# yukiteruono/pbsim3

Measured on AMD Instinct MI355X. Metric: simulated bases/sec, higher is better.
Workload: dtype u8

## Files before the change

pbsim3_amd/csrc/job.cpp:

```cpp
#include <math.h>
#include <stdio.h>
#include <stdlib.h>
#include <string.h>

#include <algorithm>
#include <atomic>
#include <chrono>
#include <condition_variable>
#include <deque>
#include <future>
#include <mutex>
#include <thread>

#include "ctx.h"
#include "handoff.h"

using namespace pbsim;

namespace {

double now_us() {
  return std::chrono::duration<double, std::micro>(std::chrono::steady_clock::now().time_since_epoch()).count();
}

constexpr double kMinBatchBases = 2.0e9;
constexpr int kRoundsPerRecord = 4;

struct Rec {
  RefDesc ref;
  int64_t quota = 0, len_total = 0, next_read = 1, spec_read = 1;
  double spec_total = 0;
  int64_t cap = 0;
  bool bulk_done = false;
  bool done = false;
  int owner = -1;
  int tail_slot = -1;
  bool tail_waiting = false;
  int64_t read_off = 0, maf_off = 0;
  int64_t tail_read = 0, tail_maf = 0;
  StatsAcc st;
  bool merged = false;
};

struct Round {
  int rec, slot;
  int64_t first, n_per;
  double mean;
  bool clear;
};

struct Worker {
  std::thread th;
  std::mutex mu;
  std::condition_variable cv, cv_idle;
  std::deque<std::function<void()>> q;
  bool stop = false, running = false;
  int active = 0;
  struct Deferred {
    int key;
    std::function<bool()> ready;
    std::function<void()> run;
  };
  std::deque<Deferred> parked;
  int n_parked = 0;
  void defer(int key, std::function<bool()> ready, std::function<void()> run) {
    parked.push_back(Deferred{key, std::move(ready), std::move(run)});
    std::lock_guard<std::mutex> lk(mu);
    n_parked++;
  }
  bool run_parked() {
    bool any = false;
    for (size_t i = 0; i < parked.size();) {
      bool first_of_key = true;
      for (size_t j = 0; j < i; j++) first_of_key &= parked[j].key != parked[i].key;
      if (first_of_key && parked[i].ready()) {
        Deferred d = std::move(parked[i]);
        parked.erase(parked.begin() + (long)i);
        d.run();
        {
          std::lock_guard<std::mutex> lk(mu);
          n_parked--;
        }
        any = true;
        i = 0;
      } else {
        i++;
      }
    }
    return any;
  }
  void start(int device) {
    running = true;
    th = std::thread([this, device]() {
      (void)hipSetDevice(device);
      for (;;) {
        std::function<void()> f;
        {
          std::unique_lock<std::mutex> lk(mu);
          if (parked.empty()) cv.wait(lk, [&] { return stop || !q.empty(); });
          else cv.wait_for(lk, std::chrono::milliseconds(1), [&] { return stop || !q.empty(); });
          if (q.empty() && parked.empty()) return;
          if (!q.empty()) {
            f = std::move(q.front());
            q.pop_front();
            active++;
          }
        }
        if (f) {
          f();
          std::lock_guard<std::mutex> lk(mu);
          active--;
        }
        if (run_parked() || f) cv_idle.notify_all();
      }
    });
  }
  void post(std::function<void()> f) {
    {
      std::lock_guard<std::mutex> lk(mu);
      q.push_back(std::move(f));
    }
    cv.notify_one();
  }
  void drain() {
    if (!running) return;
    std::unique_lock<std::mutex> lk(mu);
    cv_idle.wait(lk, [&] { return q.empty() && active == 0 && n_parked == 0; });
  }
  void finish() {
    if (!running) return;
    drain();
    {
      std::lock_guard<std::mutex> lk(mu);
      stop = true;
    }
    cv.notify_all();
    th.join();
    running = false;
  }
  ~Worker() { finish(); }
};

struct Delivery {
  int slot = -1, rec = -1;
  bool mine = false;
  int64_t n_per = 0;
  std::shared_ptr<std::promise<int>> stage1;
  std::future<int> stage1_done;
  int64_t sizes[2] = {0, 0};
  int ok1 = PBSIM_SUCCEEDED;
  double t_wait0 = 0, t_wait1 = 0;
};

struct Job {
  pbsim_ctx *c;
  const pbsim_comm *comm;
  const pbsim_record_sink *sink;
  int rank = 0, W = 1;
  bool multi = false;
  std::vector<Rec> recs;
  std::deque<Round> fifo;
  double mean = 0;
  int depth = 3;
  int interleave = 1;
  int64_t reads_walked = 0, reads_delivered = 0, rounds = 0, bases = 0, ref_bases = 0, maf_columns = 0;
  double comm_us = 0;
  double bd_wait_walk = 0, bd_finalize = 0, bd_wait_bytes = 0, bd_account = 0, bd_tail_block = 0, bd_drain = 0, bd_slot_wait = 0,
         bd_merge = 0, bd_begin = 0, bd_tail_steps = 0;
  double bd_worker_busy = 0;
  int64_t n_topup = 0, n_tail_reads = 0, n_clear_missed = 0, n_exchanges = 0;
  bool trace = false;
  double t_start = 0;
  bool peer_failed = false;
  Worker worker;
  Worker tail_worker;
  std::mutex sink_mu[2];
  std::mutex out_mu;
  std::condition_variable out_cv;
  std::atomic<bool> delivering[kMaxSlots];
  std::atomic<bool> wfailed{false};
  std::mutex werr_mu;
  std::string werr;
  std::unique_ptr<Delivery> pending;
  std::unique_ptr<std::atomic<int>[]> rec_out;
  std::unique_ptr<std::atomic<int>[]> rec_bulk;
  std::unique_ptr<std::atomic<int>[]> rec_rounds_open;
  void round_closed(int rec) {
    --rec_rounds_open[(size_t)rec];
    { std::lock_guard<std::mutex> lk(out_mu); }
    out_cv.notify_all();
  }
  std::atomic<bool> giving_up{false};
  void wait_record(int rec) {
    std::unique_lock<std::mutex> lk(out_mu);
    out_cv.wait(lk, [&] { return rec_out[(size_t)rec].load() == 0; });
  }
  void delivered_one(std::atomic<int> *out, std::atomic<int> *bulk = nullptr) {
    --*out;
    if (bulk) --*bulk;
    { std::lock_guard<std::mutex> lk(out_mu); }
    out_cv.notify_all();
  }

  Job() {
    for (auto &d : delivering) d = false;
  }

  size_t n_collected = 0;
  bool seen11 = false;
  double bd_record_wait = 0;
  const DeviceFlags *record_arrived(int i) {
    JobRecord *jr = nullptr;
    {
      std::unique_lock<std::mutex> lk(c->job_mu);
      const double t0 = now_us();
      const bool came = c->job_cv.wait_for(lk, std::chrono::seconds(600),
                                           [&] { return c->job_records.size() > (size_t)i || c->job_feed_failed; });
      bd_record_wait += now_us() - t0;
      if (c->job_records.size() <= (size_t)i) {
        fail(!came ? "pbsim_job_run: a record announced by pbsim_job_expect did not arrive within 600 s" : c->job_feed_err);
        return nullptr;
      }
      jr = c->job_records[(size_t)i].get();
    }
    const double t1 = now_us();
    if (hipEventSynchronize(jr->ready) != hipSuccess) {
      fail("hipEventSynchronize failed (a record's preparation)");
      return nullptr;
// ... 5 lines not shown
    while ((int)n_collected <= upto) {
      const size_t i = n_collected;
      const DeviceFlags *f = record_arrived((int)i);
      if (!f) return PBSIM_FAILED;
      JobRecord *jr;
      {
        std::lock_guard<std::mutex> lk(c->job_mu);
        jr = c->job_records[i].get();
      }
      if (trace) fprintf(stderr, "[pbsim job r%d] t=%.1f ms record %zu collected (waited %.1f ms for records so far)\n", rank, (now_us() - t_start) / 1e3, i + 1, bd_record_wait / 1e3);
      seen11 |= f->hpfreq[11] > 0;
      jr->ref.seq = jr->seq.as<uint8_t>();
      jr->ref.hp = jr->hp.as<uint8_t>();
      jr->ref.len = jr->len;
      jr->ref.unit = c->job_first_unit + (int64_t)i;
      jr->ref.hp_flag = c->p.hp_del_bias == 1 && !f->high_bytes;
      jr->ref.hp11 = seen11;
      recs[i].ref = jr->ref;
      c->bias.hp11_seen = seen11;
      if (!ensure_tables(c, jr->ref.hp11)) return PBSIM_FAILED;
      n_collected++;
    }
    return PBSIM_SUCCEEDED;
  }

  void worker_fail() {
    std::lock_guard<std::mutex> lk(werr_mu);
    if (!wfailed) werr = g_err;
    wfailed = true;
  }
  int check_worker() {
    if (!wfailed) return PBSIM_SUCCEEDED;
    std::lock_guard<std::mutex> lk(werr_mu);
    return fail(werr);
  }

  void progress(int phase, int rec, int64_t first = 0, int64_t n_per = 0) {
    int64_t *g = c->job_progress;
    g[0] = phase;
    g[1] = rec;
    g[2] = first;
    g[3] = n_per;
    g[4] = W;
    g[5] = rec >= 0 ? recs[(size_t)rec].len_total : 0;
    g[6] = rec >= 0 ? recs[(size_t)rec].quota : 0;
    g[7] = rec >= 0 ? recs[(size_t)rec].next_read : 0;
  }
  int gather(const int64_t *send, int64_t n, std::vector<int64_t> *recv) {
    recv->assign((size_t)W * n, 0);
    if (!multi) {
      memcpy(recv->data(), send, (size_t)n * 8);
      return PBSIM_SUCCEEDED;
    }
    const double t0 = now_us();
    const int ok = comm->all_gather_i64(comm->user, send, n, recv->data());
    comm_us += now_us() - t0;
    n_exchanges++;
    return ok ? PBSIM_SUCCEEDED : fail("pbsim_comm.all_gather_i64 failed");
  }

  bool slot_busy(int s) const {
    if (delivering[s]) return true;
    for (const Round &r : fifo)
      if (r.slot == s) return true;
    for (const Rec &r : recs)
      if (r.tail_slot == s) return true;
    return false;
  }
  static constexpr int kTailSlot = kMaxSlots - 2;
  int free_slot() const {
    for (int s = 0; s < kTailSlot; s++)
      if (!slot_busy(s)) return s;
    return -1;
  }
  int free_tail_slot() const {
    for (int s = kTailSlot; s < kMaxSlots; s++)
      if (!slot_busy(s)) return s;
    return -1;
  }
  int bulk_in_flight() const { return (int)fifo.size(); }
  int acquire_slot() {
    const double t0 = now_us();
    for (;;) {
      const int s = free_slot();
      if (s >= 0) {
        bd_slot_wait += now_us() - t0;
        return s;
      }
      std::unique_lock<std::mutex> lk(worker.mu);
      worker.cv_idle.wait_for(lk, std::chrono::milliseconds(2));
    }
  }

  void drop_round(const Round &r) {
    c->cur = r.slot;
    (void)hipStreamSynchronize(c->s().stream);
    (void)settle_slot(r.slot);
    c->s().b_enqueued = false;
  }
  void drop_rounds_of(int rec) {
    for (auto it = fifo.begin(); it != fifo.end();) {
      if (it->rec == rec) {
        drop_round(*it);
        it = fifo.erase(it);
      } else {
        ++it;
      }
    }
  }
  void drop_everything(bool failing = true) {
    if (failing) {
      giving_up = true;
      { std::lock_guard<std::mutex> lk(out_mu); }
      out_cv.notify_all();
    }
    worker.drain();
    tail_worker.drain();
    for (const Round &r : fifo) drop_round(r);
    fifo.clear();
    for (Rec &r : recs)
      if (r.tail_slot >= 0) {
        c->cur = r.tail_slot;
        (void)hipStreamSynchronize(c->s().stream);
        c->s().b_enqueued = false;
        r.tail_slot = -1;
      }
  }

  Handoff handoff;
  bool handoff_on = false;
  bool lookahead = false;
  int64_t n_handed = 0, n_handed_void = 0;
  void publish_next(int slot) {
    const Slot &sl = c->slots[slot];
    if (!handoff_on || sl.b_info.n_final <= 0) return;
    HandoffNext d;
    d.slot = slot;
    d.text[0] = sink->on_read_text ? sl.d_read_text.p : nullptr;
    d.text[1] = sink->on_maf_text ? sl.d_maf_text.p : nullptr;
    d.bytes[0] = sl.b_info.read_text_bytes;
    d.bytes[1] = sl.b_info.maf_text_bytes;
    d.ev_text = sl.ev_text;
    handoff.publish(d);
  }
  unsigned withdraw_next() {
    if (!handoff_on) return 0;
    const unsigned took = handoff.withdraw();
    n_handed += (took & 1) + (took >> 1);
    return took;
  }
  int settle_slot(int slot) {
    for (DfLane &L : c->slots[slot].df) {
      if (L.hand_open) n_handed_void++;
      if (!deflate_settle(L)) return PBSIM_FAILED;
    }
    return PBSIM_SUCCEEDED;
  }
  std::function<bool()> tail_hook(int which) {
    return [this, which]() -> bool {
      return handoff.take(which, [&](const HandoffNext &d) {
        if (!d.text[which] || d.bytes[which] <= 0) return;
        (void)deflate_handoff(c, c->slots[d.slot].df[which], which, (const uint8_t *)d.text[which], d.bytes[which], !multi,
                              (hipEvent_t)d.ev_text);
      });
    };
  }

// ... 64 lines not shown
      }, nullptr, handoff_on ? &hook : nullptr);
    });
  }
  int arena_fill(Slot &sl, int64_t *read_gz, int64_t *maf_gz) {
    const pbsim_batch_info &bi = sl.b_info;
    *read_gz = *maf_gz = 0;
    return both_lanes(sl, [&](int which) -> int {
      DfLane &L = sl.df[which];
      L.arena_reset();
      const int64_t n = which == 0 ? bi.read_text_bytes : bi.maf_text_bytes;
      auto cb = which == 0 ? sink->on_read_text : sink->on_maf_text;
      if (!cb || n == 0) return PBSIM_SUCCEEDED;
      const uint8_t *d = which == 0 ? sl.d_read_text.as<uint8_t>() : sl.d_maf_text.as<uint8_t>();
      bool oom = false;
      const std::function<char *(int64_t)> place = [&](int64_t k) -> char * {
        char *p = L.arena_reserve(k, arena_max);
        if (!p) oom = true;
        return p;
      };
      const std::function<bool()> hook = tail_hook(which);
      if (!deflate_pieces(c, L, d, n, [](const char *, int64_t) { return PBSIM_SUCCEEDED; }, &place, handoff_on ? &hook : nullptr))
        return oom ? fail("out of pinned host memory for a compressed batch (PBSIM_PINNED_ARENA_MB bounds a lane's arena)") : PBSIM_FAILED;
      int64_t tot = 0;
      for (const auto &sg : L.arena_segs) tot += sg.second;
      (which == 0 ? *read_gz : *maf_gz) = tot;
      return PBSIM_SUCCEEDED;
    });
  }
  int arena_flush(Slot &sl, int64_t unit, int64_t read_at, int64_t maf_at) {
    return both_lanes(sl, [&](int which) -> int {
      int64_t at = which == 0 ? read_at : maf_at;
      for (const auto &sg : sl.df[which].arena_segs) {
        if (!call_sink(which, unit, sg.first, sg.second, at)) return fail(which == 0 ? "sink aborted (read text)" : "sink aborted (MAF text)");
        at += sg.second;
      }
      sl.df[which].arena_segs.clear();
      return PBSIM_SUCCEEDED;
    });
  }

  void submit_stage1(Delivery *d) {
    d->stage1 = std::make_shared<std::promise<int>>();
    d->stage1_done = d->stage1->get_future();
    if (!d->mine) {
      d->stage1->set_value(PBSIM_SUCCEEDED);
      return;
    }
    delivering[d->slot] = true;
    Slot *sl = &c->slots[d->slot];
    Rec *R = &recs[(size_t)d->rec];
    auto prom = d->stage1;
    int64_t *sizes = d->sizes;
    const int64_t read_at = R->read_off, maf_at = R->maf_off;
    std::atomic<int> *out = &rec_out[(size_t)d->rec], *bulk = &rec_bulk[(size_t)d->rec];
    ++*out;
    ++*bulk;
    worker.post([this, sl, R, prom, sizes, read_at, maf_at, out, bulk]() {
      const double w0 = now_us();
      int ok = PBSIM_SUCCEEDED;
      if (wants_text() && hipEventSynchronize(sl->ev_text) != hipSuccess) ok = fail("hipEventSynchronize failed (text emission)");
      if (!ok) {
      } else if (!wants_text()) {
        sizes[0] = sizes[1] = 0;
      } else if (!deflated()) {
        ok = fetch_plain(*sl);
        sizes[0] = sink->on_read_text ? sl->b_info.read_text_bytes : 0;
        sizes[1] = sink->on_maf_text ? sl->b_info.maf_text_bytes : 0;
      } else if (!multi) {
        ok = stream_deflated(*sl, R->ref.unit, read_at, maf_at, &sizes[0], &sizes[1]);
      } else {
        ok = arena_fill(*sl, &sizes[0], &sizes[1]);
      }
      if (!ok) worker_fail();
      bd_worker_busy += now_us() - w0;
      if (trace)
        fprintf(stderr, "[pbsim job r%d] t=%.1f ms   worker: bytes of rec %lld on their way for %.1f ms (%lld + %lld)\n", rank,
                (w0 - t_start) / 1e3, (long long)R->ref.unit, (now_us() - w0) / 1e3, (long long)sizes[0], (long long)sizes[1]);
      delivered_one(out, bulk);
      prom->set_value(ok);
    });
  }
  Slot *acct_slot = nullptr;
  Rec *acct_rec = nullptr;
  int account_deferred() {
    if (!acct_slot) return PBSIM_SUCCEEDED;
    Slot *sl = acct_slot;
    acct_slot = nullptr;
    const double t0 = now_us();
    const int ok = account_of(c, *sl, &acct_rec->st);
    bd_account += now_us() - t0;
    round_closed((int)(acct_rec - recs.data()));
    return ok;
  }
  int wait_pending(int64_t c3[3]) {
    c3[0] = c3[1] = c3[2] = 0;
    if (!pending) return PBSIM_SUCCEEDED;
    const double t0 = now_us();
    const int ok1 = pending->stage1_done.get();
    pending->ok1 = ok1;
    pending->t_wait0 = t0;
    pending->t_wait1 = now_us();
    bd_wait_bytes += pending->t_wait1 - t0;
    c3[0] = pending->mine ? pending->sizes[0] : 0;
    c3[1] = pending->mine ? pending->sizes[1] : 0;
    c3[2] = ok1 ? 0 : 1;
    return PBSIM_SUCCEEDED;
  }
  int apply_pending(const std::vector<int64_t> &S, int stride, int at, bool defer_account) {
    if (!pending) return PBSIM_SUCCEEDED;
    std::unique_ptr<Delivery> d = std::move(pending);
    Rec &R = recs[(size_t)d->rec];
    const int ok1 = d->ok1;
    int64_t read_at = R.read_off, maf_at = R.maf_off, read_all = 0, maf_all = 0, bad = 0;
    for (int q = 0; q < W; q++) {
      const int64_t *v = &S[(size_t)q * stride + at];
      if (q < rank) {
        read_at += v[0];
        maf_at += v[1];
      }
      read_all += v[0];
      maf_all += v[1];
      bad += v[2];
    }
    if (bad) {
      if (ok1) peer_failed = true;
      return ok1 ? fail("another rank of the job failed") : check_worker();
    }
    R.read_off += read_all;
    R.maf_off += maf_all;
    if (d->mine) {
      Slot *sl = &c->slots[d->slot];
      Rec *Rp = &R;
      const int slot = d->slot;
      const bool flush = deflated() && multi, plain = wants_text() && !deflated();
      acct_slot = sl;
      acct_rec = &R;
      std::atomic<int> *out = &rec_out[(size_t)d->rec], *bulk = &rec_bulk[(size_t)d->rec];
      if (flush || plain) {
        ++*out;
        ++*bulk;
      }
      if (!defer_account && !account_deferred()) return PBSIM_FAILED;
      if (flush || plain) {
        worker.post([this, sl, Rp, slot, flush, read_at, maf_at, out, bulk]() {
          const int ok = flush ? arena_flush(*sl, Rp->ref.unit, read_at, maf_at) : sink_plain(*sl, Rp->ref.unit, read_at, maf_at);
          if (!ok) worker_fail();
          delivering[slot] = false;
          delivered_one(out, bulk);
        });
      } else {
        delivering[slot] = false;
      }
    } else {
      round_closed(d->rec);
    }
    if (trace)
      fprintf(stderr, "[pbsim job r%d] t=%.1f ms rec %d delivery: waited %.1f ms for the bytes (%lld + %lld)\n", rank,
              (d->t_wait0 - t_start) / 1e3, d->rec + 1, (d->t_wait1 - d->t_wait0) / 1e3, (long long)d->sizes[0], (long long)d->sizes[1]);
    return check_worker();
  }
  int complete_pending(bool defer_account = false) {
    if (!account_deferred()) return PBSIM_FAILED;
    if (!pending) return PBSIM_SUCCEEDED;
    int64_t mine2[3];
    if (!wait_pending(mine2)) return PBSIM_FAILED;
    std::vector<int64_t> S;
    progress(3, pending->rec, 0, pending->n_per);
    if (!gather(mine2, 3, &S)) return PBSIM_FAILED;
    return apply_pending(S, 3, 0, defer_account);
  }

  int tail_begin(Rec &R) {
    const int s = free_tail_slot();
    if (s < 0) {
      R.tail_waiting = true;
      return PBSIM_SUCCEEDED;
    }
    R.tail_waiting = false;
    c->cur = s;
    const int64_t remaining = R.quota - R.len_total;
    if (!walk_begin(c, R.ref, R.next_read, chain_reads_for(c, R.ref.len, remaining), remaining, true)) return PBSIM_FAILED;
    R.tail_slot = s;
    return PBSIM_SUCCEEDED;
  }
  int tail_poll(int rec, bool block) {
    Rec &R = recs[(size_t)rec];
    for (;;) {
      if (R.tail_waiting) {
        if (block) {
          for (size_t o = 0; o < recs.size(); o++)
            if ((int)o != rec && recs[o].tail_slot >= 0 && !tail_poll((int)o, true)) return PBSIM_FAILED;
          const double t_wait = now_us();
          while (free_tail_slot() < 0 && !wfailed && !giving_up) {
            std::unique_lock<std::mutex> lk(tail_worker.mu);
            tail_worker.cv_idle.wait_for(lk, std::chrono::milliseconds(1));
            if (now_us() - t_wait > 120e6) return fail("internal: the chains of truncated reads hold both slots and none comes back (120 s)");
          }
        }
        if (!tail_begin(R)) return PBSIM_FAILED;
        if (R.tail_waiting) return block ? fail("internal: no slot for the truncated reads") : PBSIM_SUCCEEDED;
      }
      if (R.tail_slot < 0) return PBSIM_SUCCEEDED;
      c->cur = R.tail_slot;
      if (!block && hipEventQuery(c->s().ev3) != hipSuccess) return PBSIM_SUCCEEDED;
      const double t0 = now_us();
      pbsim_batch_info bi;
      if (!chain_end_finalize(c, R.len_total, &bi)) return PBSIM_FAILED;
      n_tail_reads += bi.n_final;
      const int slot = R.tail_slot;
      Slot *sl = &c->slots[slot];
      Rec *Rp = &R;
      delivering[slot] = true;
      std::atomic<int> *out = &rec_out[(size_t)rec];
      ++*out;
      tail_worker.post([this, sl, Rp, slot, out, rec]() {
        int ok = PBSIM_SUCCEEDED;
        std::string zr, zm;
        const pbsim_batch_info &bi2 = sl->b_info;
        if (wants_text() && hipEventSynchronize(sl->ev_text) != hipSuccess) ok = fail("hipEventSynchronize failed (text emission)");
        if (!ok) {
        } else if (deflated()) {
          ok = both_lanes(*sl, [&](int which) -> int {
            const int64_t n = which == 0 ? bi2.read_text_bytes : bi2.maf_text_bytes;
            if (!(which == 0 ? sink->on_read_text : sink->on_maf_text) || n == 0) return PBSIM_SUCCEEDED;
            std::string *z = which == 0 ? &zr : &zm;
            const uint8_t *d = which == 0 ? sl->d_read_text.as<uint8_t>() : sl->d_maf_text.as<uint8_t>();
            return deflate_pieces(c, sl->df[which], d, n, [z](const char *p, int64_t k) {
              z->append(p, (size_t)k);
              return PBSIM_SUCCEEDED;
            });
          });
        } else if (wants_text()) {
          ok = fetch_plain(*sl);
        }
        if (!ok) worker_fail();
        const std::string err1 = ok ? std::string() : g_err;
        auto members = std::make_shared<std::pair<std::string, std::string>>(std::move(zr), std::move(zm));
        tail_worker.defer(
            rec,
            [this, rec]() {
              return wfailed.load() || giving_up.load() ||
                     (rec_rounds_open[(size_t)rec].load() == 0 && (!wants_text() || rec_bulk[(size_t)rec].load() == 0));
            },
            [this, sl, Rp, slot, out, ok, members]() {
              int ok2 = ok && !giving_up && !wfailed;
              const int64_t read_at = Rp->read_off + Rp->tail_read, maf_at = Rp->maf_off + Rp->tail_maf;
              int64_t nr = 0, nm = 0;
              if (!ok2) {
              } else if (deflated()) {
                nr = (int64_t)members->first.size();
                nm = (int64_t)members->second.size();
                if (nr && !call_sink(0, Rp->ref.unit, members->first.data(), nr, read_at)) ok2 = fail("sink aborted (read text)");
                if (ok2 && nm && !call_sink(1, Rp->ref.unit, members->second.data(), nm, maf_at)) ok2 = fail("sink aborted (MAF text)");
              } else if (wants_text()) {
                ok2 = sink_plain(*sl, Rp->ref.unit, read_at, maf_at);
                nr = sink->on_read_text ? sl->b_info.read_text_bytes : 0;
                nm = sink->on_maf_text ? sl->b_info.maf_text_bytes : 0;
              }
              if (ok2) ok2 = account_of(c, *sl, &Rp->st);
              Rp->tail_read += nr;
              Rp->tail_maf += nm;
              if (ok && !ok2 && !giving_up && !wfailed) worker_fail();
              delivering[slot] = false;
              delivered_one(out);
            });
      });
      reads_walked += bi.n_final;
      reads_delivered += bi.n_final;
      bases += bi.bases;
      ref_bases += bi.ref_bases;
      maf_columns += bi.maf_columns;
      if (trace)
        fprintf(stderr, "[pbsim job r%d] t=%.1f ms rec %d tail chain from read %lld: %lld reads, %.2f ms to collect\n", rank,
                (t0 - t_start) / 1e3, rec + 1, (long long)R.next_read, (long long)bi.n_final, (now_us() - t0) / 1e3);
      R.next_read += bi.n_final;
      R.len_total = bi.len_total_after;
      R.tail_slot = -1;
      if (!block) bd_tail_steps += now_us() - t0;
      if (R.len_total < R.quota) {
        if (!tail_begin(R)) return PBSIM_FAILED;
      } else {
        R.done = true;
        return PBSIM_SUCCEEDED;
      }
    }
  }

  int finish_record(int rec) {
    Rec &R = recs[(size_t)rec];
    if (pending && pending->rec == rec && !complete_pending()) return PBSIM_FAILED;
    if (!account_deferred()) return PBSIM_FAILED;
    const double tt = now_us();
    int tail_ok = PBSIM_SUCCEEDED;
    std::string tail_err;
    if (rank == R.owner && !tail_poll(rec, true)) {
      tail_ok = PBSIM_FAILED;
      tail_err = g_err;
    }
    const double td = now_us();
    bd_tail_block += td - tt;
    wait_record(rec);
    bd_drain += now_us() - td;
    int64_t extra[3] = {R.tail_read, R.tail_maf, (tail_ok && !wfailed) ? 0 : 1};
    const double t0 = now_us();
    progress(4, rec);
    if (!stats_merge(&R.st, c->p, multi ? comm : nullptr, extra, 3)) return PBSIM_FAILED;
    bd_merge += now_us() - t0;
    if (!tail_ok) return fail(tail_err);
    if (!check_worker()) return PBSIM_FAILED;
    if (extra[2]) {
      peer_failed = true;
      return fail("another rank of the job failed");
    }
    R.merged = R.done = true;
    pbsim_stats st;
    stats_finish(R.st, c->p, R.ref.len, &st);
    c->st = R.st;
    c->st.blocks.clear();
    R.st = StatsAcc();
    if (sink && sink->on_record_done &&
        !sink->on_record_done(sink->user, recs[(size_t)rec].ref.unit, &st, R.read_off + extra[0], R.maf_off + extra[1]))
      return fail("sink aborted (record done)");
    return PBSIM_SUCCEEDED;
  }

  int begin_round(int rec) {
    Rec &R = recs[(size_t)rec];
    const double remaining = (double)R.quota - R.spec_total;
    int64_t n_total = (int64_t)(1.005 * remaining / mean) + 64;
    if (remaining <= 0) n_total = 64;
    int64_t n_per = std::min<int64_t>((n_total + W - 1) / W, R.cap);
    if (rounds < 2) n_per = std::min<int64_t>(n_per, std::max<int64_t>(64, (int64_t)((double)R.cap * (rounds == 0 ? 0.2 : 0.5))));
    n_per = std::max<int64_t>(n_per, 1);
    if (!collect(rec)) return PBSIM_FAILED;
    const int s = acquire_slot();
    c->cur = s;
    if (!settle_slot(s)) return PBSIM_FAILED;
    const double tb = now_us();
    if (trace) fprintf(stderr, "[pbsim job r%d] begin rec %d first=%lld n_per=%lld\n", rank, rec + 1, (long long)R.spec_read, (long long)n_per);
    if (!walk_begin(c, R.ref, R.spec_read + (int64_t)rank * n_per, n_per, -1)) return PBSIM_FAILED;
    bd_begin += now_us() - tb;
    const double after = R.spec_total + (double)W * (double)n_per * mean;
    const char *force_clear = getenv("PBSIM_JOB_CLEAR");
    const bool clear = force_clear ? atoi(force_clear) != 0
                                   : (double)R.quota - after > 0.04 * (double)W * (double)n_per * mean + 2.0 * (double)std::min<int64_t>(c->p.len_max, R.ref.len);
    fifo.push_back(Round{rec, s, R.spec_read, n_per, mean, clear});
    R.spec_read += (int64_t)W * n_per;
    R.spec_total += (double)W * (double)n_per * mean;
    reads_walked += n_per;
    rounds++;
    return PBSIM_SUCCEEDED;
  }

  static constexpr int kMsg = 8;
  int process_round() {
    const Round rd = fifo.front();
    fifo.pop_front();
    Rec &R = recs[(size_t)rd.rec];
    c->cur = rd.slot;
    struct Withdraw {
      Job *j;
      ~Withdraw() { (void)j->withdraw_next(); }
    } withdraw_at_exit{this};
    const double t0 = now_us();
    int64_t pass0 = 0, code = 0;
    std::string my_err;
    if (!pbsim_batch_walk_end(c, &pass0)) {
      my_err = g_err;
      code = (my_err.rfind("scratch budget exceeded", 0) == 0 && rd.n_per > 1) ? 1 : 2;
    }
    if (wfailed) code = 2;
    const double t1 = now_us();
    bd_wait_walk += t1 - t0;
    for (size_t r = 0; r < recs.size(); r++)
      if ((recs[r].tail_slot >= 0 || recs[r].tail_waiting) && !tail_poll((int)r, false)) return PBSIM_FAILED;
    c->cur = rd.slot;
    const int64_t max_raw = c->s().b_max_raw;
    pbsim_batch_info bi;
    memset(&bi, 0, sizeof bi);
    int fin_ok = PBSIM_SUCCEEDED;
    double t_fin = 0;
    std::vector<int64_t> A, B;
    int64_t msg[kMsg] = {pass0, code, max_raw, 0, 0, 0, 0, 0};
    bool c_applied = false;
    if (rd.clear) {
      if (code == 0) {
        const double tf = now_us();
        fin_ok = finalize_uncut(c, &bi) && finalize_text(c, &bi);
        if (!fin_ok) my_err = g_err;
        else publish_next(rd.slot);
        t_fin += now_us() - tf;
      }
      msg[3] = fin_ok ? 0 : 1;
      if (pending) {
        msg[4] = 1;
        if (!wait_pending(&msg[5])) return PBSIM_FAILED;
      }
      progress(6, rd.rec, rd.first, rd.n_per);
      if (!gather(msg, kMsg, &A)) return PBSIM_FAILED;
      c_applied = true;
    } else {
      progress(1, rd.rec, rd.first, rd.n_per);
      if (!gather(msg, kMsg, &A)) return PBSIM_FAILED;
    }
    int64_t worst = 0, pass0_sum = 0, before = R.len_total, raw_all = 0, bad_fin = 0;
    for (int q = 0; q < W; q++) {
      worst = std::max(worst, A[(size_t)q * kMsg + 1]);
      pass0_sum += A[(size_t)q * kMsg];
      raw_all = std::max(raw_all, A[(size_t)q * kMsg + 2]);
      bad_fin += A[(size_t)q * kMsg + 3];
      if (q < rank) before += A[(size_t)q * kMsg];
    }
    if (c_applied && worst != 2 && !apply_pending(A, kMsg, 5, true)) return PBSIM_FAILED;
    if (worst == 2 || (worst == 0 && bad_fin)) {
      drop_everything();
      if (wfailed) return check_worker();
      if (code != 2 && fin_ok) peer_failed = true;
      return fail(code == 2 || !fin_ok ? my_err : "another rank of the job failed");
    }
    if (worst == 1) {
      if (!complete_pending()) return PBSIM_FAILED;
      drop_everything(false);
// ... 40 lines not shown
        drop_everything();
        if (fin_ok) peer_failed = true;
        return fail(fin_ok ? "another rank of the job failed" : my_err);
      }
    }
    bd_finalize += t_fin;
    const double t2 = now_us();
    int cut = -1;
    for (int q = 0; q < W && cut < 0; q++)
      if (B[(size_t)q * kMsg] < rd.n_per) cut = q;
    const int last_valid = cut < 0 ? W - 1 : cut;
    const bool mine = rank <= last_valid && bi.n_final > 0;
    if (!c_applied && !complete_pending(true)) return PBSIM_FAILED;
    const unsigned handed = withdraw_next();
    if (trace && handoff_on)
      fprintf(stderr, "[pbsim job r%d] t=%.1f ms rec %d hand-off: %s%s%s\n", rank, (now_us() - t_start) / 1e3, rd.rec + 1,
              handed == 0 ? "no lane took the round" : (handed == 3 ? "both lanes' heads launched" : "one lane's head launched"),
              handed ? " behind the round in front" : "", handed && !mine ? " (void: the block is behind the cut)" : "");
    pending.reset(new Delivery);
    ++rec_rounds_open[(size_t)rd.rec];
    pending->slot = rd.slot;
    pending->rec = rd.rec;
    pending->mine = mine;
    pending->n_per = rd.n_per;
    submit_stage1(pending.get());
    if (!account_deferred()) return PBSIM_FAILED;
    if (mine) {
      reads_delivered += bi.n_final;
      bases += bi.bases;
      ref_bases += bi.ref_bases;
      maf_columns += bi.maf_columns;
    }
    const double t3 = now_us();
    const double n_round = (double)W * (double)rd.n_per;
    R.spec_total += (double)pass0_sum - n_round * rd.mean;
    if (n_round >= 1000) {
      const double measured = (double)pass0_sum / n_round;
      for (Round &pr : fifo) {
        recs[(size_t)pr.rec].spec_total += (double)W * (double)pr.n_per * (measured - pr.mean);
        pr.mean = measured;
      }
      mean = measured;
    }
    if (cut < 0) {
      R.next_read += (int64_t)W * rd.n_per;
      R.len_total = B[(size_t)(W - 1) * kMsg + 2];
    } else {
      R.next_read += (int64_t)cut * rd.n_per + B[(size_t)cut * kMsg];
      R.len_total = B[(size_t)cut * kMsg + 2];
      R.spec_read = R.next_read;
      R.spec_total = (double)R.len_total;
      if (B[(size_t)cut * kMsg + 1] && R.len_total < R.quota) {
        R.owner = cut;
        R.bulk_done = true;
      }
    }
    if (R.len_total >= R.quota) R.bulk_done = true;
    if (R.bulk_done) {
      drop_rounds_of(rd.rec);
      if (rank == R.owner) {
        if (!tail_begin(R)) return PBSIM_FAILED;
      } else {
        R.done = true;
      }
    }
    if (trace)
      fprintf(stderr,
              "[pbsim job r%d] t=%.1f ms rec %d round first=%lld n=%lldx%d %s final=%lld cut=%d wait_walk=%.1f finalize=%.1f handover=%.1f "
              "comm=%.1f ms\n",
              rank, (t0 - t_start) / 1e3, rd.rec + 1, (long long)rd.first, (long long)rd.n_per, W,
              rd.clear ? (untouched ? "clear" : "clear-missed") : "cutting", (long long)bi.n_final, cut, (t1 - t0) / 1e3, t_fin / 1e3,
              (t3 - t2) / 1e3, comm_us / 1e3);
    return PBSIM_SUCCEEDED;
  }

  int run() {
    const int n = (int)recs.size();
    int merged = 0;
    worker.start(c->device);
    tail_worker.start(c->device);
    for (;;) {
      if (!check_worker()) return PBSIM_FAILED;
      const int open_max = std::max(2, interleave);
      auto depth_now = [&]() {
        if (!lookahead || depth != 1 || fifo.size() != 1) return depth;
        const Round &r = fifo.front();
        return 4 * r.n_per <= recs[(size_t)r.rec].cap ? 2 : 1;
      };
      while (bulk_in_flight() < depth_now()) {
        int cand = -1;
        const int hi = std::min(n, merged + open_max);
        double best = 2.0;
        for (int r = merged; r < hi; r++) {
          const Rec &R = recs[(size_t)r];
          if (R.bulk_done || (double)R.quota - R.spec_total <= 0) continue;
          if (interleave <= 1) {
            cand = r;
            break;
          }
          const double f = R.spec_total / (double)std::max<int64_t>(1, R.quota);
          if (f < best) {
            best = f;
            cand = r;
          }
        }
        if (cand < 0) {
          for (int r = merged; r < hi && cand < 0; r++) {
            bool has = false;
            for (const Round &pr : fifo) has |= pr.rec == r;
            if (!recs[(size_t)r].bulk_done && !has) cand = r;
          }
          if (cand >= 0) n_topup++;
        }
        if (cand < 0) {
          if (hi >= n) break;
          if (!recs[(size_t)merged].bulk_done) break;
          if (!finish_record(merged)) return PBSIM_FAILED;
          merged++;
          continue;
        }
        if (!begin_round(cand)) return PBSIM_FAILED;
      }
      for (int r = 0; r < n; r++)
        if ((recs[(size_t)r].tail_slot >= 0 || recs[(size_t)r].tail_waiting) && !tail_poll(r, false)) return PBSIM_FAILED;
      if (fifo.empty()) {
        for (int r = 0; r < n; r++)
          if (!recs[(size_t)r].bulk_done) return fail("internal: a record lacks reads but nothing is in flight");
        break;
      }
      if (!process_round()) return PBSIM_FAILED;
    }
    for (; merged < n; merged++) {
      if (!recs[(size_t)merged].bulk_done) return fail("internal: a record was left unfinished");
      if (!finish_record(merged)) return PBSIM_FAILED;
    }
    if (!complete_pending()) return PBSIM_FAILED;
    worker.finish();
    tail_worker.finish();
    return check_worker();
  }
};

}

extern "C" {

static int job_publish(pbsim_ctx *c, std::unique_ptr<JobRecord> r) {
  if (!r->h_flags) HIP_OK(hipHostMalloc((void **)&r->h_flags, sizeof(DeviceFlags), hipHostMallocDefault));
  HIP_OK(hipMemcpyAsync(r->h_flags, r->flags.p, sizeof(DeviceFlags), hipMemcpyDeviceToHost, c->prefetch_stream));
  HIP_OK(hipEventCreateWithFlags(&r->ready, hipEventDisableTiming));
  HIP_OK(hipEventRecord(r->ready, c->prefetch_stream));
  {
    std::lock_guard<std::mutex> lk(c->job_mu);
    const size_t i = c->job_records.size();
    if (!c->job_expect_len.empty() && (i >= c->job_expect_len.size() || c->job_expect_len[i] != r->len)) {
      c->job_feed_failed = true;
      c->job_feed_err = "pbsim_job_add_record: not the record pbsim_job_expect announced (count or length)";
      c->job_cv.notify_all();
      return fail(c->job_feed_err);
    }
    c->job_records.push_back(std::move(r));
  }
  c->job_cv.notify_all();
  return PBSIM_SUCCEEDED;
}

static std::unique_ptr<JobRecord> job_new_record(pbsim_ctx *c, int64_t len) {
  {
    std::lock_guard<std::mutex> lk(c->job_mu);
    for (size_t i = 0; i < c->job_spare.size(); i++)
      if (c->job_spare[i]->len == len && c->job_spare[i]->seq.bytes >= (size_t)len + 64) {
        std::unique_ptr<JobRecord> r = std::move(c->job_spare[i]);
        c->job_spare.erase(c->job_spare.begin() + (long)i);
        r->ref = RefDesc();
        return r;
      }
    for (size_t i = c->job_spare.size(); i-- > 0;) {
      bool wanted = false;
      for (size_t k = c->job_records.size(); k < c->job_expect_len.size() && !wanted; k++)
        wanted = c->job_expect_len[k] == c->job_spare[i]->len;
      if (!wanted) c->job_spare.erase(c->job_spare.begin() + (long)i);
    }
  }
  std::unique_ptr<JobRecord> r(new JobRecord);
  r->len = len;
  return r;
}

static int job_add(pbsim_ctx *c, const void *seq, int64_t len, hipMemcpyKind kind) {
  if (!c || !seq) return fail("pbsim_job_add_record: bad argument");
  const bool trace = getenv("PBSIM_TRACE") != nullptr;
  const double ta = now_us();
  NEED_DEVICE(c);
  if (c->p.strategy != PBSIM_STRATEGY_WGS || c->p.method == PBSIM_METHOD_SAMPLE)
    return fail("pbsim_job_add_record: the job pipeline runs --strategy wgs with --method errhmm or qshmm");
  if (len < 1) return fail("Reference is too short.");
  if (len > 1000000000LL) return fail("Reference is too long. Acceptable length <= 1000000000.");
  HIP_OK(hipSetDevice(c->device));
  if (!c->prefetch_stream) HIP_OK(hipStreamCreateWithFlags(&c->prefetch_stream, hipStreamNonBlocking));
  std::unique_ptr<JobRecord> r = job_new_record(c, len);
  HIP_OK(r->seq.ensure((size_t)len + 64, true));
  HIP_OK(hipMemcpyAsync(r->seq.p, seq, (size_t)len, kind, c->prefetch_stream));
// ... 278 lines not shown
  if (!c->scratch_factor_fixed && c->need_seen == 0) {
    c->cur = 0;
    for (int64_t n_probe = std::min<int64_t>(8192, batch_capacity_for(c, J.recs[0].ref.len)); n_probe >= 32; n_probe /= 4) {
      if (!walk_begin(c, J.recs[0].ref, 1, n_probe, -1)) return PBSIM_FAILED;
      const int ok = pbsim_batch_walk_end(c, nullptr);
      c->s().b_walked = false;
      if (ok) break;
      if (g_err.rfind("scratch budget exceeded", 0) != 0) return PBSIM_FAILED;
    }
  }
  const double sf = scratch_factor_of(c);
  const int P = c->p.pass_num;
  const int regions = has_quality(c) ? 3 : 2;
  const bool delivers_text = sink && (sink->on_read_text || sink->on_maf_text);
  const int rounds_per_record = delivers_text ? (multi ? 2 : kRoundsPerRecord) : 2;
  double target = (double)max_quota * P / ((double)rounds_per_record * W);
  target = std::max(target, std::min(kMinBatchBases, (double)max_quota * P / W));
  if (J.sink && (J.sink->on_read_text || J.sink->on_maf_text)) target = std::min(target, kSinkBatchBases);
  if (c->scratch_auto) {
    size_t free_b = 0, total_b = 0;
    HIP_OK(hipMemGetInfo(&free_b, &total_b));
    if (streaming) {
      std::lock_guard<std::mutex> lk(c->job_mu);
      std::vector<int64_t> spare;
      for (auto &sp : c->job_spare) spare.push_back(sp->len);
      size_t pending = 0, lines_max = 0;
      for (size_t i = 0; i < n; i++) {
        if (i < c->job_records.size()) {
          free_b += (size_t)(2 * lens[i] + 192);
        }
        auto it = std::find(spare.begin(), spare.end(), lens[i]);
        if (it != spare.end() && i >= c->job_records.size()) {
          spare.erase(it);
          continue;
        }
        pending += (size_t)(2 * lens[i] + 192) + (size_t)(lens[i] / 1024 + 64) * 16;
        lines_max = std::max(lines_max, (size_t)(lens[i] + lens[i] / 40 + 64));
      }
      if (c->d_lines.bytes > 0 && lines_max > c->d_lines.bytes) pending += lines_max - c->d_lines.bytes;
      free_b = free_b > pending ? free_b - pending : 0;
    }
    size_t held = 0, held_text = 0;
    for (Slot &sl : c->slots) {
      held += sl.d_scratch.bytes;
      held_text += sl.d_read_text.bytes + sl.d_maf_text.bytes;
    }
    {
      const double text_per_base = 1.125 * ((P > 1 ? (c->bam_output ? 5.8 : 8.4) : 4.25) + (c->truth_bam ? 0.2 : 0.0));
      const double scratch_per_base = (double)regions * sf * 1.12 * 1.08 + 0.1;
      const bool delivering_text = J.sink && (J.sink->on_read_text || J.sink->on_maf_text);
      const double slots_used = (double)J.depth + (delivering_text ? 3.0 : 1.0);
      const char *ff = getenv("PBSIM_JOB_FIT");
      const double fit = (ff ? atof(ff) : 0.75) * (double)(free_b + held + held_text) / (slots_used * (text_per_base + scratch_per_base));
      target = std::min(target, std::max(fit, 1.0e8));
    }
    const double mean_len = std::max(1.0, c->hdr.mean_len);
    const double want = (target / P / mean_len) * P * ((double)regions * (sf * mean_len + kScratchPad) * 1.12 + 64.0) * 1.08 + (64 << 20);
    const double share = std::min(48.0 * (1LL << 30), 0.14 * (double)(free_b + held));
    const int64_t auto_b = (int64_t)std::max(256.0 * (1 << 20), std::min(want, share));
    if ((double)auto_b > 1.10 * (double)c->scratch_budget || c->scratch_budget > 2 * auto_b) c->scratch_budget = auto_b;
  }
  if (const char *tr = getenv("PBSIM_JOB_TARGET_RANKS")) {
    std::vector<double> v;
    for (const char *q = tr; *q;) {
      char *e = nullptr;
      v.push_back(strtod(q, &e));
      if (e == q) break;
      q = *e == ',' ? e + 1 : e;
    }
    if (!v.empty() && v[(size_t)J.rank % v.size()] > 0) target = v[(size_t)J.rank % v.size()];
  }
  std::vector<int64_t> agree(n + 1);
  agree[0] = c->scratch_budget;
  J.progress(5, -1);
  if (multi) {
    if (!comm->all_reduce_i64(comm->user, agree.data(), 1, PBSIM_OP_MIN)) return fail("pbsim_comm.all_reduce_i64 failed");
    c->scratch_budget = agree[0];
  }
  J.mean = 0.97 * c->hdr.mean_len;
  for (size_t i = 0; i < n; i++) {
    Rec &R = J.recs[i];
    const double m = std::min<double>(c->hdr.mean_len, (double)R.ref.len);
    R.cap = std::max<int64_t>(1, std::min<int64_t>(batch_capacity_for(c, R.ref.len), (int64_t)(1.08 * target / P / m) + 64));
    agree[i + 1] = R.cap;
  }
  if (multi) {
    if (!comm->all_reduce_i64(comm->user, agree.data(), (int64_t)agree.size(), PBSIM_OP_MIN)) return fail("pbsim_comm.all_reduce_i64 failed");
    for (size_t i = 0; i < n; i++) J.recs[i].cap = agree[i + 1];
  }
  J.mean = std::min<double>(J.mean, (double)lens[0]);
  for (Slot &sl : c->slots) sl.b_enqueued = sl.b_walked = sl.b_finalized = false;
  {
    const char *am = getenv("PBSIM_PINNED_ARENA_MB");
    J.arena_max = (size_t)(am && atoll(am) > 0 ? atoll(am) : 16384) << 20;
  }
  int ready = (!J.deflated() || ensure_deflate_ready(c)) ? PBSIM_SUCCEEDED : PBSIM_FAILED;
  if (multi) {
    const std::string keep = g_err;
    int64_t bad = ready ? 0 : 1;
    if (!comm->all_reduce_i64(comm->user, &bad, 1, PBSIM_OP_MAX)) return fail("pbsim_comm.all_reduce_i64 failed");
    if (bad) {
      *settled = true;
      return ready ? fail("another rank of the job failed") : fail(keep);
    }
  } else if (!ready) {
    return PBSIM_FAILED;
  }
  const int keep_lds = c->walk_lds_kb;
  if (J.deflated()) c->walk_lds_kb = std::max(c->walk_lds_kb, 81);
  c->defer_text_sync = true;
  {
    const char *ho = getenv("PBSIM_JOB_HANDOFF");
    J.handoff_on = J.deflated() && c->deflate_parallel && !(ho && atoi(ho) == 0);
    const char *la = getenv("PBSIM_JOB_LOOKAHEAD");
    J.lookahead = delivers && !(la && atoi(la) == 0);
  }
  if (J.trace) fprintf(stderr, "[pbsim job r%d] entered at %.3f ms, round loop at %.3f ms\n", J.rank, J.t_start / 1e3, now_us() / 1e3);
  int ok = J.run();
  c->defer_text_sync = false;
  c->walk_lds_kb = keep_lds;
  for (Slot &sl : c->slots)
    if (sl.stream && hipStreamSynchronize(sl.stream) != hipSuccess && ok) ok = fail("hipStreamSynchronize failed at the end of the job");
  if (!ok) {
    const std::string keep = g_err;
    if (multi && !J.peer_failed && comm->abort) comm->abort(comm->user);
    *settled = true;
    J.drop_everything();
    J.worker.finish();
    J.tail_worker.finish();
    g_err = keep;
  }
  (void)J.withdraw_next();
  for (int s = 0; s < kMaxSlots; s++)
    if (!J.settle_slot(s) && ok) ok = PBSIM_FAILED;
  for (Slot &sl : c->slots)
    for (DfLane &L : sl.df) L.arena_trim();
  if (J.trace)
    fprintf(stderr, "[pbsim job r%d] returns at %.3f ms; hand-off %s: %lld lane heads launched at a tail, %lld of them never delivered\n",
            J.rank, now_us() / 1e3, J.handoff_on ? "on" : "off", (long long)J.n_handed, (long long)J.n_handed_void);
  {
    const double wall = now_us() - J.t_start;
    double *b = c->job_breakdown;
    b[0] = wall;
    b[1] = J.bd_wait_walk;
    b[2] = J.bd_finalize;
    b[3] = J.bd_wait_bytes;
    b[4] = J.comm_us;
    b[5] = J.bd_account;
    b[6] = J.bd_tail_block;
    b[7] = J.bd_drain;
    b[8] = J.bd_slot_wait + J.bd_record_wait;
    b[9] = J.bd_merge;
    b[10] = J.bd_begin;
    b[11] = J.bd_tail_steps;
    b[12] = J.bd_worker_busy;
    b[13] = (double)J.n_topup;
    b[14] = (double)J.n_tail_reads;
    b[15] = (double)J.depth;
  }
  c->job_counters[0] = J.reads_walked;
  c->job_counters[1] = J.reads_delivered;
  c->job_counters[2] = J.rounds;
  c->job_counters[3] = J.bases;
  c->job_counters[4] = (int64_t)(now_us() - J.t_start);
  c->job_counters[5] = (int64_t)J.comm_us;
  c->job_counters[6] = J.ref_bases;
  c->job_counters[7] = J.maf_columns;
  return ok;
}

int pbsim_job_run(pbsim_ctx *c, const pbsim_comm *comm, const pbsim_record_sink *sink) {
  if (!c) return fail("bad argument");
  NEED_DEVICE(c);
  if (comm && (comm->world < 1 || comm->rank < 0 || comm->rank >= comm->world)) return fail("pbsim_comm: bad rank / world");
  if (comm && comm->world > 1 && (!comm->all_gather_i64 || !comm->all_reduce_i64))
    return fail("pbsim_comm: all_gather_i64 and all_reduce_i64 must be set");
  bool settled = false;
  const int ok = job_run_impl(c, comm, sink, &settled);
  if (!ok && !settled && comm && comm->world > 1 && comm->abort) {
    const std::string keep = g_err;
    comm->abort(comm->user);
    g_err = keep;
  }
  return ok;
}

int64_t pbsim_format_stats(const pbsim_params *p, const pbsim_stats *s, int64_t unit, char *buf, int64_t cap) {
  if (!p || !s) return -1;
  char t[1024];
  int k = 0;
  if (p->strategy == PBSIM_STRATEGY_WGS) {
    k += snprintf(t + k, sizeof t - k, ":::: Simulation stats (ref.%ld) ::::\n\n", (long)unit);
    k += snprintf(t + k, sizeof t - k, "read num. : %ld\n", (long)s->res_num);
    k += snprintf(t + k, sizeof t - k, "depth : %lf\n", s->res_depth);
  } else {
    k += snprintf(t + k, sizeof t - k, ":::: Simulation stats ::::\n\n");
    k += snprintf(t + k, sizeof t - k, "read num. : %ld\n", (long)s->res_num);
  }
  k += snprintf(t + k, sizeof t - k, "read length mean (SD) : %f (%f)\n", s->res_len_mean, s->res_len_sd);
  k += snprintf(t + k, sizeof t - k, "read length min : %ld\n", (long)s->res_len_min);
  k += snprintf(t + k, sizeof t - k, "read length max : %ld\n", (long)s->res_len_max);
  k += snprintf(t + k, sizeof t - k, "read accuracy mean (SD) : %f (%f)\n", s->res_accuracy_mean, s->res_accuracy_sd);
  k += snprintf(t + k, sizeof t - k, "substitution rate. : %f\n", s->res_sub_rate);
  k += snprintf(t + k, sizeof t - k, "insertion rate. : %f\n", s->res_ins_rate);
  k += snprintf(t + k, sizeof t - k, "deletion rate. : %f\n", s->res_del_rate);
  k += snprintf(t + k, sizeof t - k, "\n");
  if (buf && cap > k) memcpy(buf, t, (size_t)k + 1);
  return k;
}

}
```

Measured before the change: 58.34 billion.

## Ramp round sizes geometrically and overlap rounds, accounting and tail walks more aggressively

Replaces the two-step ramp of round sizes with a geometric ramp starting at cap/16 with a per-read-length floor. A second round may now begin beside a small one. Pending rounds are accounted early and tail walks start before the pending delivery completes. The walk's LDS size is chosen per round depending on whether the deflate link is idle, and slot acquisition avoids unallocated slots while others still deliver. This adds scheduling complexity and a trace-only NUMA probe; the smaller early rounds may add per-round overhead.

```diff
diff --git a/pbsim3_amd/csrc/job.cpp b/pbsim3_amd/csrc/job.cpp
--- a/pbsim3_amd/csrc/job.cpp
+++ b/pbsim3_amd/csrc/job.cpp
@@ -2,6 +2,8 @@
 #include <stdio.h>
 #include <stdlib.h>
 #include <string.h>
+#include <sys/syscall.h>
+#include <unistd.h>
 
 #include <algorithm>
 #include <atomic>
@@ -14,6 +16,7 @@
 
 #include "ctx.h"
 #include "handoff.h"
+#include "round_plan.h"
 
 using namespace pbsim;
 
@@ -21,6 +24,19 @@
 
 double now_us() {
   return std::chrono::duration<double, std::micro>(std::chrono::steady_clock::now().time_since_epoch()).count();
+}
+
+int numa_node_of(const void *p) {
+#ifdef SYS_move_pages
+  if (!p) return -1;
+  void *page = (void *)((uintptr_t)p & ~(uintptr_t)4095);
+  int status = -1;
+  if (syscall(SYS_move_pages, 0, 1UL, &page, nullptr, &status, 0) != 0) return -1;
+  return status;
+#else
+  (void)p;
+  return -1;
+#endif
 }
 
 constexpr double kMinBatchBases = 2.0e9;
@@ -31,6 +47,7 @@
   int64_t quota = 0, len_total = 0, next_read = 1, spec_read = 1;
   double spec_total = 0;
   int64_t cap = 0;
+  int64_t ramp_floor = 0;
   bool bulk_done = false;
   bool done = false;
   int owner = -1;
@@ -144,6 +161,7 @@
 struct Delivery {
   int slot = -1, rec = -1;
   bool mine = false;
+  bool accounted = false;
   int64_t n_per = 0;
   std::shared_ptr<std::promise<int>> stage1;
   std::future<int> stage1_done;
@@ -315,7 +333,14 @@
   int acquire_slot() {
     const double t0 = now_us();
     for (;;) {
-      const int s = free_slot();
+      int s = free_slot();
+      if (s >= 0 && c->slots[s].d_scratch.bytes == 0) {
+        for (int t = 0; t < kTailSlot && s >= 0; t++) {
+          bool with_loop = pending && pending->slot == t;
+          for (const Round &r : fifo) with_loop |= r.slot == t;
+          if (delivering[t] && !with_loop && c->slots[t].d_scratch.bytes > 0) s = -1;
+        }
+      }
       if (s >= 0) {
         bd_slot_wait += now_us() - t0;
         return s;
@@ -546,14 +571,25 @@
   }
   Slot *acct_slot = nullptr;
   Rec *acct_rec = nullptr;
+  bool acct_taken = false;
   int account_deferred() {
     if (!acct_slot) return PBSIM_SUCCEEDED;
     Slot *sl = acct_slot;
     acct_slot = nullptr;
     const double t0 = now_us();
-    const int ok = account_of(c, *sl, &acct_rec->st);
+    const int ok = acct_taken ? PBSIM_SUCCEEDED : account_of(c, *sl, &acct_rec->st);
+    acct_taken = false;
     bd_account += now_us() - t0;
     round_closed((int)(acct_rec - recs.data()));
+    return ok;
+  }
+  int account_pending_early() {
+    if (!pending || !pending->mine || pending->accounted) return PBSIM_SUCCEEDED;
+    if (!account_deferred()) return PBSIM_FAILED;
+    const double t0 = now_us();
+    const int ok = account_of(c, c->slots[pending->slot], &recs[(size_t)pending->rec].st);
+    bd_account += now_us() - t0;
+    pending->accounted = true;
     return ok;
   }
   int wait_pending(int64_t c3[3]) {
@@ -599,6 +635,7 @@
       const bool flush = deflated() && multi, plain = wants_text() && !deflated();
       acct_slot = sl;
       acct_rec = &R;
+      acct_taken = d->accounted;
       std::atomic<int> *out = &rec_out[(size_t)d->rec], *bulk = &rec_bulk[(size_t)d->rec];
       if (flush || plain) {
         ++*out;
@@ -643,13 +680,16 @@
     R.tail_waiting = false;
     c->cur = s;
     const int64_t remaining = R.quota - R.len_total;
+    c->walk_lds_kb = walk_lds_beside_deflate;
     if (!walk_begin(c, R.ref, R.next_read, chain_reads_for(c, R.ref.len, remaining), remaining, true)) return PBSIM_FAILED;
     R.tail_slot = s;
     return PBSIM_SUCCEEDED;
   }
-  int tail_poll(int rec, bool block) {
+  static constexpr int kTailEarly = 2;
+  int tail_poll(int rec, int block) {
     Rec &R = recs[(size_t)rec];
     for (;;) {
+      if (R.tail_waiting && block == kTailEarly && free_tail_slot() < 0) return PBSIM_SUCCEEDED;
       if (R.tail_waiting) {
         if (block) {
           for (size_t o = 0; o < recs.size(); o++)
@@ -752,12 +792,19 @@
 
   int finish_record(int rec) {
     Rec &R = recs[(size_t)rec];
-    if (pending && pending->rec == rec && !complete_pending()) return PBSIM_FAILED;
+    int tail_ok = PBSIM_SUCCEEDED;
+    std::string tail_err;
+    if (pending && pending->rec == rec) {
+      if (!account_pending_early()) return PBSIM_FAILED;
+      if (rank == R.owner && !tail_poll(rec, kTailEarly)) {
+        tail_ok = PBSIM_FAILED;
+        tail_err = g_err;
+      }
+      if (!complete_pending()) return PBSIM_FAILED;
+    }
     if (!account_deferred()) return PBSIM_FAILED;
     const double tt = now_us();
-    int tail_ok = PBSIM_SUCCEEDED;
-    std::string tail_err;
-    if (rank == R.owner && !tail_poll(rec, true)) {
+    if (tail_ok && rank == R.owner && !tail_poll(rec, true)) {
       tail_ok = PBSIM_FAILED;
       tail_err = g_err;
     }
@@ -788,20 +835,32 @@
     return PBSIM_SUCCEEDED;
   }
 
-  int begin_round(int rec) {
-    Rec &R = recs[(size_t)rec];
+  int64_t next_n_per(int rec) const {
+    const Rec &R = recs[(size_t)rec];
     const double remaining = (double)R.quota - R.spec_total;
     int64_t n_total = (int64_t)(1.005 * remaining / mean) + 64;
     if (remaining <= 0) n_total = 64;
-    int64_t n_per = std::min<int64_t>((n_total + W - 1) / W, R.cap);
-    if (rounds < 2) n_per = std::min<int64_t>(n_per, std::max<int64_t>(64, (int64_t)((double)R.cap * (rounds == 0 ? 0.2 : 0.5))));
-    n_per = std::max<int64_t>(n_per, 1);
+    return round_plan::round_size(rounds, R.cap, n_total, W, R.ramp_floor);
+  }
+  bool link_idle() const {
+    return !pending || !pending->mine || !pending->stage1_done.valid() || pending->stage1_done.wait_for(std::chrono::seconds(0)) == std::future_status::ready;
+  }
+  int walk_lds_free = 27, walk_lds_beside_deflate = 27;
+  int begin_round(int rec) {
+    Rec &R = recs[(size_t)rec];
+    const int64_t n_per = next_n_per(rec);
     if (!collect(rec)) return PBSIM_FAILED;
     const int s = acquire_slot();
     c->cur = s;
     if (!settle_slot(s)) return PBSIM_FAILED;
     const double tb = now_us();
-    if (trace) fprintf(stderr, "[pbsim job r%d] begin rec %d first=%lld n_per=%lld\n", rank, rec + 1, (long long)R.spec_read, (long long)n_per);
+    const bool idle = fifo.empty() && link_idle();
+    c->walk_lds_kb = idle ? walk_lds_free : walk_lds_beside_deflate;
+    if (trace) {
+      fprintf(stderr, "[pbsim job r%d] begin rec %d first=%lld n_per=%lld\n", rank, rec + 1, (long long)R.spec_read, (long long)n_per);
+      fprintf(stderr, "[pbsim job r%d] walk of rec %d first=%lld lds=%d%s\n", rank, rec + 1, (long long)R.spec_read, c->walk_lds_kb,
+              idle ? " (idle link)" : "");
+    }
     if (!walk_begin(c, R.ref, R.spec_read + (int64_t)rank * n_per, n_per, -1)) return PBSIM_FAILED;
     bd_begin += now_us() - tb;
     const double after = R.spec_total + (double)W * (double)n_per * mean;
@@ -1008,12 +1067,15 @@
     for (;;) {
       if (!check_worker()) return PBSIM_FAILED;
       const int open_max = std::max(2, interleave);
-      auto depth_now = [&]() {
-        if (!lookahead || depth != 1 || fifo.size() != 1) return depth;
-        const Round &r = fifo.front();
-        return 4 * r.n_per <= recs[(size_t)r.rec].cap ? 2 : 1;
-      };
-      while (bulk_in_flight() < depth_now()) {
+      for (;;) {
+        const int in_flight = bulk_in_flight();
+        const bool beside = in_flight >= depth;
+        if (beside && (fifo.empty() || round_plan::rounds_allowed(lookahead, depth, in_flight, 0, 1, 1) <= in_flight)) break;
+        auto allowed = [&](int rec) {
+          if (!beside) return true;
+          const Round &f = fifo.front();
+          return round_plan::rounds_allowed(lookahead, depth, in_flight, f.n_per, next_n_per(rec), recs[(size_t)f.rec].cap) > in_flight;
+        };
         int cand = -1;
         const int hi = std::min(n, merged + open_max);
         double best = 2.0;
@@ -1030,20 +1092,29 @@
             cand = r;
           }
         }
+        bool topup = false;
         if (cand < 0) {
           for (int r = merged; r < hi && cand < 0; r++) {
             bool has = false;
             for (const Round &pr : fifo) has |= pr.rec == r;
             if (!recs[(size_t)r].bulk_done && !has) cand = r;
           }
-          if (cand >= 0) n_topup++;
+          topup = cand >= 0;
         }
         if (cand < 0) {
           if (hi >= n) break;
           if (!recs[(size_t)merged].bulk_done) break;
+          if (!allowed(hi)) break;
           if (!finish_record(merged)) return PBSIM_FAILED;
           merged++;
           continue;
+        }
+        if (!allowed(cand)) break;
+        if (topup) n_topup++;
+        if (beside && trace) {
+          const Round &f = fifo.front();
+          fprintf(stderr, "[pbsim job r%d] rec %d round of n_per=%lld begun beside the round of n_per=%lld of rec %d (cap %lld)\n", rank,
+                  cand + 1, (long long)next_n_per(cand), (long long)f.n_per, f.rec + 1, (long long)recs[(size_t)f.rec].cap);
         }
         if (!begin_round(cand)) return PBSIM_FAILED;
       }
@@ -1488,6 +1559,7 @@
     Rec &R = J.recs[i];
     const double m = std::min<double>(c->hdr.mean_len, (double)R.ref.len);
     R.cap = std::max<int64_t>(1, std::min<int64_t>(batch_capacity_for(c, R.ref.len), (int64_t)(1.08 * target / P / m) + 64));
+    R.ramp_floor = round_plan::ramp_floor(m);
     agree[i + 1] = R.cap;
   }
   if (multi) {
@@ -1513,7 +1585,9 @@
     return PBSIM_FAILED;
   }
   const int keep_lds = c->walk_lds_kb;
-  if (J.deflated()) c->walk_lds_kb = std::max(c->walk_lds_kb, 81);
+  J.walk_lds_free = keep_lds;
+  J.walk_lds_beside_deflate = J.deflated() ? std::max(keep_lds, 81) : keep_lds;
+  c->walk_lds_kb = J.walk_lds_beside_deflate;
   c->defer_text_sync = true;
   {
     const char *ho = getenv("PBSIM_JOB_HANDOFF");
@@ -1541,6 +1615,15 @@
     if (!J.settle_slot(s) && ok) ok = PBSIM_FAILED;
   for (Slot &sl : c->slots)
     for (DfLane &L : sl.df) L.arena_trim();
+  if (J.trace && J.deflated()) {
+    std::string where;
+    for (int s = 0; s < Job::kTailSlot; s++)
+      for (int w = 0; w < 2; w++)
+        for (int k = 0; k < kDfBuffers; k++)
+          if (c->slots[s].df[w].h_df_out[k].p)
+            where += " " + std::to_string(s) + "." + std::to_string(w) + "." + std::to_string(k) + ":" + std::to_string(numa_node_of(c->slots[s].df[w].h_df_out[k].p));
+    fprintf(stderr, "[pbsim job r%d] NUMA node of the lanes' pinned staging (slot.lane.buffer:node)%s\n", J.rank, where.c_str());
+  }
   if (J.trace)
     fprintf(stderr, "[pbsim job r%d] returns at %.3f ms; hand-off %s: %lld lane heads launched at a tail, %lld of them never delivered\n",
             J.rank, now_us() / 1e3, J.handoff_on ? "on" : "off", (long long)J.n_handed, (long long)J.n_handed_void);
diff --git a/pbsim3_amd/csrc/round_plan.h b/pbsim3_amd/csrc/round_plan.h
--- /dev/null
+++ b/pbsim3_amd/csrc/round_plan.h
@@ -0,0 +1,38 @@
+#pragma once
+#include <stdint.h>
+
+#include <algorithm>
+
+namespace pbsim {
+namespace round_plan {
+
+constexpr int64_t kRampFirstDiv = 16;
+constexpr int64_t kRampGrowth = 2;
+constexpr int64_t kRampFloor = 64;
+constexpr int64_t kRampFloorBases = 1000000;
+inline int64_t ramp_floor(double mean_len) {
+  return std::max<int64_t>(kRampFloor, (int64_t)((double)kRampFloorBases / std::max(mean_len, 1.0)));
+}
+
+inline int64_t round_size(int64_t rounds_begun, int64_t cap, int64_t n_total, int64_t W, int64_t floor = kRampFloor) {
+  cap = std::max<int64_t>(cap, 1);
+  W = std::max<int64_t>(W, 1);
+  const int64_t want = std::max<int64_t>((std::max<int64_t>(n_total, 0) + W - 1) / W, 1);
+  if (want <= cap) return want;
+  int64_t div = kRampFirstDiv;
+  for (int64_t k = 0; k < rounds_begun && div > 1; k++) div /= kRampGrowth;
+  return std::min(std::max<int64_t>(floor, cap / std::max<int64_t>(div, 1)), cap);
+}
+
+constexpr int64_t kBesidePct = 45;
+inline bool begin_beside(int64_t front_n_per, int64_t next_n_per, int64_t cap) {
+  return 4 * front_n_per <= cap || 100 * front_n_per <= kBesidePct * next_n_per;
+}
+
+inline int rounds_allowed(bool lookahead, int depth, int in_flight, int64_t front_n_per, int64_t next_n_per, int64_t cap) {
+  if (!lookahead || depth != 1 || in_flight != 1) return depth;
+  return begin_beside(front_n_per, next_n_per, cap) ? 2 : 1;
+}
+
+}
+}
```

New measurement: 59.22 billion, median of 6. 1.02x the previous value.
